# svohr/mixemt

Hardware: AMD Instinct MI355X
Metric: read x hap cells/sec through the EM iteration (EM iters/sec reported beside it as em_iters_per_s), 1000000 reads x 5408 haps in total, whole job (higher is better)
Workload: dtype f64

## Files before the change

### include/mixemt_hip_tuning.h

```cpp
#ifndef MIXEMT_HIP_TUNING_H
#define MIXEMT_HIP_TUNING_H

#include <stddef.h>
#include <stdint.h>

#ifdef __cplusplus
extern "C" {
#endif

struct mxm_em_state;

int mxm_reset_tuning(void);

int mxm_set_timing_events(void *ev_start, void *ev_stop);

int mxm_describe_stream_kernel(int32_t H, int32_t nb, char *buf, size_t len);

int mxm_diag_stream_read(const void *src, size_t bytes, int32_t wg_per_cu, int32_t blocked,
                         void *sink, void *stream);

struct mxm_coded;
int mxm_diag_stream_coded(const struct mxm_coded *c, int32_t H, int32_t wg_per_cu, void *sink, void *stream);

int mxm_diag_stream_quads(const struct mxm_coded *c, int32_t H, int32_t wg_per_cu, void *sink, void *stream);

int mxm_set_progress_callback(void (*fn)(const struct mxm_em_state *state_host, int32_t B, void *user),
                              void *user, int32_t every);

int mxm_set_loop_graph(int32_t mode);

int mxm_set_loop_fused(int32_t mode, int32_t chunk);

int mxm_set_fused_coded_grid(int32_t nwg);

int mxm_set_quad_left_grid(int32_t nwg);

int mxm_set_sparse_long_rows(int32_t on);
int mxm_set_sparse_long_entries(int32_t n);

int mxm_set_quad_encoder(int32_t kind);

int mxm_set_coded_batch_tile(int32_t bt);

int mxm_diag_fused_force_abort(int32_t on);

int mxm_diag_fused_stamps(const void *ws, unsigned long long *out_host);

int mxm_set_batch_tile(int32_t bt);

int mxm_set_compact_restarts(int32_t mode);

int mxm_set_min_rows_per_wg(int32_t n);

int mxm_set_sparse_max_distinct(int32_t n);

#ifdef __cplusplus
}
#endif
#endif
```

### mixemt_amd/_lib.py

```python

import ctypes
import os

_PKG = os.path.dirname(os.path.abspath(__file__))
LIB_PATH = os.environ.get("MXM_LIB") or os.path.join(_PKG, "lib", "libmixemt_hip.so")

c_i32, c_i64, c_f64 = ctypes.c_int32, ctypes.c_int64, ctypes.c_double
c_ptr, c_size = ctypes.c_void_p, ctypes.c_size_t


class EmState(ctypes.Structure):
    _fields_ = [("done", c_i32), ("iters", c_i32), ("l1", c_f64), ("ticket", ctypes.c_uint32), ("error", ctypes.c_uint32)]


class Coded(ctypes.Structure):
    _fields_ = [("rec", c_ptr), ("rec_off", c_ptr), ("ndist", c_ptr), ("R", c_i64),
                ("P_rest", c_ptr), ("ldp_rest", c_i64), ("w_rest", c_ptr), ("R_rest", c_i64),
                ("wide_rows", c_ptr), ("n_wide", c_i64),
                ("qrec", c_ptr), ("qoff", c_ptr), ("nquad", c_ptr), ("quad_rows", c_ptr), ("n_quad_rows", c_i64),
                ("byte_rows", c_ptr), ("n_byte_rows", c_i64)]


class AlnColumns(ctypes.Structure):
    _fields_ = [("n_aln", c_i64), ("n_frag", c_i64), ("ref_start", c_ptr), ("mapq", c_ptr), ("frag", c_ptr),
# ... 36 lines not shown
    "mxm_linearize": (ctypes.c_int, [c_ptr, c_i64, c_i64, c_i32, c_ptr, c_i64, c_ptr, c_ptr]),
    "mxm_em_iter": (ctypes.c_int, [c_ptr, c_i64, c_ptr, c_i64, c_ptr, c_ptr, c_ptr, c_i64, c_i32, c_i32,
                                   c_ptr, c_ptr, c_ptr, c_size, c_ptr]),
    "mxm_m_finalize": (ctypes.c_int, [c_ptr, c_ptr, c_ptr, c_ptr, c_i32, c_i32, c_f64, c_i32, c_ptr,
                                      c_ptr]),
    "mxm_em_loop": (ctypes.c_int, [c_ptr, c_i64, c_ptr, c_i64, c_ptr, c_i64, c_i32, c_i32,
                                   c_ptr, c_ptr, c_ptr, c_ptr, c_ptr, c_f64, c_i32, c_i32, c_ptr, c_size,
                                   c_ptr, ctypes.POINTER(EmState)]),
    "mxm_linearize_f32": (ctypes.c_int, [c_ptr, c_i64, c_i64, c_i32, c_ptr, c_i64, c_ptr, c_ptr]),
    "mxm_em_iter_f32": (ctypes.c_int, [c_ptr, c_i64, c_ptr, c_ptr, c_i64, c_i32, c_i32, c_ptr, c_ptr, c_ptr,
                                       c_size, c_ptr]),
    "mxm_em_loop_f32": (ctypes.c_int, [c_ptr, c_i64, c_ptr, c_i64, c_i32, c_i32, c_ptr, c_ptr, c_ptr, c_ptr,
                                       c_ptr, c_f64, c_i32, c_i32, c_ptr, c_size, c_ptr,
                                       ctypes.POINTER(EmState)]),
    "mxm_coded_bytes": (c_size, [c_i64, c_i32]),
    "mxm_exchange_handle_bytes": (c_size, []),
    "mxm_exchange_create": (ctypes.c_int, [c_i32, c_i32, c_i64, ctypes.POINTER(c_ptr), c_ptr]),
    "mxm_exchange_connect": (ctypes.c_int, [c_ptr, c_ptr]),
    "mxm_exchange_push": (ctypes.c_int, [c_ptr, c_ptr, c_i64, c_ptr]),
    "mxm_exchange_pull": (ctypes.c_int, [c_ptr, c_ptr, c_i64, c_ptr, c_i32, c_ptr]),
    "mxm_exchange_reduce": (ctypes.c_int, [c_ptr, c_ptr, c_i64, c_ptr, c_i32, c_ptr]),
    "mxm_exchange_info": (ctypes.c_int, [c_ptr, ctypes.POINTER(c_i32), ctypes.POINTER(c_i64)]),
    "mxm_exchange_destroy": (None, [c_ptr]),
    "mxm_expand_tables": (ctypes.c_int, [c_ptr, c_ptr, c_ptr, c_ptr, c_ptr, c_i32, c_i32, c_i64, c_ptr, c_ptr]),
    "mxm_quad_bytes": (c_size, [c_i64, c_i32]),
    "mxm_quad_lists_scratch_bytes": (c_size, [c_i64]),
    "mxm_quad_lists": (ctypes.c_int, [c_ptr, c_ptr, c_i64, c_ptr, c_ptr, c_ptr, c_ptr, c_size, c_ptr]),
    "mxm_build_quads": (ctypes.c_int, [ctypes.POINTER(Coded), c_i32, c_ptr, c_size, c_ptr, c_ptr, c_ptr, c_ptr]),
    "mxm_encode_rows": (ctypes.c_int, [c_ptr, c_i64, c_i64, c_i32, c_ptr, c_size, c_ptr, c_ptr, c_ptr, c_ptr, c_ptr]),
    "mxm_decode_rows": (ctypes.c_int, [ctypes.POINTER(Coded), c_i32, c_ptr, c_i64, c_ptr]),
    "mxm_row_argmax_votes_coded": (ctypes.c_int, [ctypes.POINTER(Coded), c_i32, c_i32, c_ptr, c_ptr, c_ptr, c_ptr, c_i64,
                                                  c_ptr, c_i64, c_ptr, c_ptr, c_ptr, c_ptr, c_size, c_ptr]),
    "mxm_em_step_coded": (ctypes.c_int, [ctypes.POINTER(Coded), c_i32, c_ptr, c_ptr, c_ptr, c_ptr, c_i64, c_ptr, c_i64,
                                         c_ptr, c_i64, c_i32, c_ptr]),
    "mxm_gather_columns_coded": (ctypes.c_int, [ctypes.POINTER(Coded), c_i32, c_ptr, c_i32, c_ptr, c_i64, c_ptr, c_i64,
                                                c_ptr, c_i64, c_ptr]),
    "mxm_em_iter_coded": (ctypes.c_int, [ctypes.POINTER(Coded), c_ptr, c_ptr, c_i32, c_i32, c_ptr, c_ptr, c_ptr,
                                         c_size, c_ptr]),
    "mxm_em_loop_coded": (ctypes.c_int, [ctypes.POINTER(Coded), c_ptr, c_i32, c_i32, c_ptr, c_ptr, c_ptr, c_ptr,
                                         c_ptr, c_f64, c_i32, c_i32, c_ptr, c_size, c_ptr,
                                         ctypes.POINTER(EmState)]),
    "mxm_em_step": (ctypes.c_int, [c_ptr, c_i64, c_ptr, c_ptr, c_i64, c_i32, c_ptr, c_i64, c_i32,
                                   c_ptr, c_ptr, c_size, c_ptr]),
    "mxm_log_normalize": (ctypes.c_int, [c_ptr, c_i32, c_ptr, c_ptr]),
    "mxm_l1_exp_diff": (ctypes.c_int, [c_ptr, c_ptr, c_i32, c_ptr, c_ptr]),
    "mxm_add_scalar": (ctypes.c_int, [c_ptr, c_i64, c_i64, c_i32, c_f64, c_ptr]),
    "mxm_assign_reads": (ctypes.c_int, [c_ptr, c_i64, c_ptr, c_ptr, c_i32, c_i64, c_i32, c_f64, c_ptr, c_ptr]),
    "mxm_diag_stream_read": (ctypes.c_int, [c_ptr, c_size, c_i32, c_i32, c_ptr, c_ptr]),
    "mxm_diag_stream_coded": (ctypes.c_int, [ctypes.POINTER(Coded), c_i32, c_i32, c_ptr, c_ptr]),
    "mxm_diag_stream_quads": (ctypes.c_int, [ctypes.POINTER(Coded), c_i32, c_i32, c_ptr, c_ptr]),
    "mxm_diag_fused_force_abort": (ctypes.c_int, [c_i32]),
    "mxm_set_fused_coded_grid": (ctypes.c_int, [c_i32]),
    "mxm_set_quad_left_grid": (ctypes.c_int, [c_i32]),
    "mxm_set_coded_batch_tile": (ctypes.c_int, [c_i32]),
    "mxm_set_sparse_long_rows": (ctypes.c_int, [c_i32]),
    "mxm_set_quad_encoder": (ctypes.c_int, [c_i32]),
    "mxm_set_sparse_long_entries": (ctypes.c_int, [c_i32]),
    "mxm_diag_fused_stamps": (ctypes.c_int, [c_ptr, ctypes.POINTER(ctypes.c_ulonglong)]),
    "mxm_set_timing_events": (ctypes.c_int, [c_ptr, c_ptr]),
    "mxm_set_batch_tile": (ctypes.c_int, [c_i32]),
    "mxm_encode_signatures": (ctypes.c_int64, [ctypes.c_char_p, c_ptr, c_i64, c_ptr, c_i64, c_ptr, c_ptr, c_ptr,
                                               c_i64]),
    "mxm_aln_encode": (ctypes.c_int, [ctypes.POINTER(AlnColumns), c_ptr, c_i64, c_ptr, c_i32, c_i32, c_i32, c_i32,
                                      ctypes.POINTER(c_ptr)]),
    "mxm_aln_sizes_of": (ctypes.c_int, [c_ptr, ctypes.POINTER(AlnSizes)]),
    "mxm_aln_fetch": (ctypes.c_int, [c_ptr, c_ptr, c_ptr, c_ptr, c_ptr, c_ptr, c_ptr, c_ptr, c_ptr, c_ptr]),
    "mxm_aln_fetch_fragments": (ctypes.c_int, [c_ptr, c_ptr, c_ptr, c_ptr, c_ptr]),
    "mxm_aln_free": (None, [c_ptr]),
    "mxm_bam_read": (ctypes.c_int, [ctypes.c_char_p, c_i32, ctypes.POINTER(c_ptr)]),
    "mxm_bam_sizes_of": (ctypes.c_int, [c_ptr, ctypes.POINTER(BamSizes)]),
    "mxm_bam_columns": (ctypes.c_int, [c_ptr, ctypes.POINTER(AlnColumns)]),
    "mxm_bam_fetch_names": (ctypes.c_int, [c_ptr, c_ptr, c_ptr, c_ptr, c_ptr]),
    "mxm_bam_free": (None, [c_ptr]),
    "mxm_observe_bases": (ctypes.c_int, [ctypes.POINTER(AlnColumns), c_ptr, c_i32, c_i32, c_i64, c_ptr, c_ptr]),
    "mxm_observe_bases_labelled": (ctypes.c_int, [ctypes.POINTER(AlnColumns), c_ptr, c_ptr, c_i32, c_i32, c_i32, c_i64,
                                                  c_ptr, c_ptr]),
    "mxm_consensus": (ctypes.c_int, [c_ptr, c_i32, c_i64, c_i64, c_i64, c_i32, c_ptr, c_ptr, c_ptr, c_ptr]),
    "mxm_new_variants": (ctypes.c_int, [c_ptr, c_i64, c_i32, ctypes.POINTER(c_i32), c_i32, c_i64, c_ptr, c_ptr, c_ptr]),
    "mxm_first_observed": (ctypes.c_int, [ctypes.POINTER(AlnColumns), c_ptr, c_ptr, c_i32, c_i32, c_i32, c_i64, c_ptr,
                                          c_ptr, c_ptr]),
    "mxm_extend_assign": (ctypes.c_int, [ctypes.POINTER(AlnColumns), c_ptr, c_ptr, c_i32, c_i32, ctypes.POINTER(c_i32),
                                         c_i32, c_i32, c_i32, c_i32, c_ptr, c_i64, c_ptr, c_ptr, c_ptr, c_ptr]),
    "mxm_set_compact_restarts": (ctypes.c_int, [c_i32]),
    "mxm_set_loop_graph": (ctypes.c_int, [c_i32]),
    "mxm_set_loop_fused": (ctypes.c_int, [c_i32, c_i32]),
    "mxm_set_progress_callback": (ctypes.c_int, [c_ptr, c_ptr, c_i32]),
    "mxm_set_min_rows_per_wg": (ctypes.c_int, [c_i32]),
    "mxm_reset_tuning": (ctypes.c_int, []),
    "mxm_describe_stream_kernel": (ctypes.c_int, [c_i32, c_i32, ctypes.c_char_p, c_size]),
    "mxm_set_sparse_max_distinct": (ctypes.c_int, [c_i32]),
    "mxm_row_argmax_votes": (ctypes.c_int, [c_ptr, c_i64, c_ptr, c_i64, c_i32, c_ptr, c_ptr,
                                            c_ptr, c_size, c_ptr]),
    "mxm_first_seen": (ctypes.c_int, [c_ptr, c_i64, c_i32, c_ptr, c_ptr]),
    "mxm_gather_columns": (ctypes.c_int, [c_ptr, c_i64, c_i64, c_i32, c_ptr, c_i32, c_ptr, c_i64, c_ptr]),
    "mxm_fold_logaddexp": (ctypes.c_int, [c_ptr, c_i64, ctypes.POINTER(c_ptr), ctypes.POINTER(c_i64), c_i32,
                                          c_i64, c_i32, c_f64, c_ptr]),
}

ABI_VERSION = 603

PROGRESS_FN = ctypes.CFUNCTYPE(None, ctypes.POINTER(EmState), c_i32, c_ptr)

_lib = None


class MixemtHipError(RuntimeError):
# ... 44 lines not shown
```

### mixemt_amd/csrc/common.hpp

```cpp
#ifndef MIXEMT_COMMON_HPP
#define MIXEMT_COMMON_HPP

typedef double d2 __attribute__((ext_vector_type(2)));

#define MXM_MAX_WG 1024
#define MXM_MAX_BT 4

struct mxm_slots {
    int s[MXM_MAX_BT];
};
#define MXM_LINEAR_MIN_H 65

static thread_local char g_err[512] = "";

static int fail(int code, const char *fmt, const char *a = "", long long b = 0, long long c = 0) {
    snprintf(g_err, sizeof(g_err), fmt, a, b, c);
    return code;
}
#define HIP_TRY(expr)                                                                        \
    do {                                                                                     \
        hipError_t e_ = (expr);                                                              \
        if (e_ != hipSuccess) return fail(-2, "HIP error: %s (line %lld)", hipGetErrorString(e_), __LINE__); \
    } while (0)

// ... 38 lines not shown
    return r;
}

template <int CTRL>
__device__ __forceinline__ double dpp_mov_f64(double v) {
    int lo = __double2loint(v), hi = __double2hiint(v);
    lo = __builtin_amdgcn_mov_dpp(lo, CTRL, 0xf, 0xf, true);
    hi = __builtin_amdgcn_mov_dpp(hi, CTRL, 0xf, 0xf, true);
    return __hiloint2double(hi, lo);
}
__device__ __forceinline__ double readlane_f64(double v, int src_lane) {
    const int lo = __builtin_amdgcn_readlane(__double2loint(v), src_lane);
    const int hi = __builtin_amdgcn_readlane(__double2hiint(v), src_lane);
    return __hiloint2double(hi, lo);
}
template <int CTRL, int ROW_MASK>
__device__ __forceinline__ double dpp_mov_old_f64(double old, double v) {
    int lo = __double2loint(v), hi = __double2hiint(v);
    lo = __builtin_amdgcn_update_dpp(__double2loint(old), lo, CTRL, ROW_MASK, 0xf, false);
    hi = __builtin_amdgcn_update_dpp(__double2hiint(old), hi, CTRL, ROW_MASK, 0xf, false);
    return __hiloint2double(hi, lo);
}
__device__ __forceinline__ double wave_sum_lane63(double v) {
    v += dpp_mov_f64<0xB1>(v);
    v += dpp_mov_f64<0x4E>(v);
    v += dpp_mov_f64<0x141>(v);
    v += dpp_mov_f64<0x140>(v);
    v += dpp_mov_old_f64<0x142, 0xA>(0.0, v);
    v += dpp_mov_old_f64<0x143, 0xC>(0.0, v);
    return v;
}
__device__ __forceinline__ double swap32_add(double x, double y) {
    typedef unsigned int u2s __attribute__((ext_vector_type(2)));
    const u2s lo = __builtin_amdgcn_permlane32_swap((unsigned)__double2loint(x), (unsigned)__double2loint(y), false, false);
    const u2s hi = __builtin_amdgcn_permlane32_swap((unsigned)__double2hiint(x), (unsigned)__double2hiint(y), false, false);
    return __hiloint2double((int)hi.x, (int)lo.x) + __hiloint2double((int)hi.y, (int)lo.y);
}
__device__ __forceinline__ double swap16_add(double x, double y) {
    typedef unsigned int u2s __attribute__((ext_vector_type(2)));
    const u2s lo = __builtin_amdgcn_permlane16_swap((unsigned)__double2loint(x), (unsigned)__double2loint(y), false, false);
    const u2s hi = __builtin_amdgcn_permlane16_swap((unsigned)__double2hiint(x), (unsigned)__double2hiint(y), false, false);
    return __hiloint2double((int)hi.x, (int)lo.x) + __hiloint2double((int)hi.y, (int)lo.y);
}
__device__ __forceinline__ double wave_sum3_by_row(double a, double b, double c) {
    const double ab = swap32_add(a, b);
    const double cc = swap32_add(c, c);
    double v = swap16_add(ab, cc);
    v += dpp_mov_f64<0xB1>(v);
    v += dpp_mov_f64<0x4E>(v);
    v += dpp_mov_f64<0x141>(v);
    v += dpp_mov_f64<0x140>(v);
    return v;
}
__device__ __forceinline__ double wave_max_lane63(double v) {
    v = fmax(v, dpp_mov_f64<0xB1>(v));
    v = fmax(v, dpp_mov_f64<0x4E>(v));
    v = fmax(v, dpp_mov_f64<0x141>(v));
    v = fmax(v, dpp_mov_f64<0x140>(v));
    v = fmax(v, dpp_mov_old_f64<0x142, 0xA>(v, v));
    v = fmax(v, dpp_mov_old_f64<0x143, 0xC>(v, v));
    return v;
}

__device__ __forceinline__ int wave_min_lane63_i32(int v) {
    v = min(v, __builtin_amdgcn_mov_dpp(v, 0xB1, 0xf, 0xf, true));
    v = min(v, __builtin_amdgcn_mov_dpp(v, 0x4E, 0xf, 0xf, true));
    v = min(v, __builtin_amdgcn_mov_dpp(v, 0x141, 0xf, 0xf, true));
    v = min(v, __builtin_amdgcn_mov_dpp(v, 0x140, 0xf, 0xf, true));
    v = min(v, __builtin_amdgcn_update_dpp(v, v, 0x142, 0xA, 0xf, false));
    v = min(v, __builtin_amdgcn_update_dpp(v, v, 0x143, 0xC, 0xf, false));
    return v;
}

__device__ __forceinline__ int wave_inclusive_scan_i32(int v) {
    v += __builtin_amdgcn_update_dpp(0, v, 0x111, 0xf, 0xf, false);
    v += __builtin_amdgcn_update_dpp(0, v, 0x112, 0xf, 0xf, false);
    v += __builtin_amdgcn_update_dpp(0, v, 0x114, 0xf, 0xf, false);
    v += __builtin_amdgcn_update_dpp(0, v, 0x118, 0xf, 0xf, false);
    v += __builtin_amdgcn_update_dpp(0, v, 0x142, 0xa, 0xf, false);
    v += __builtin_amdgcn_update_dpp(0, v, 0x143, 0xc, 0xf, false);
    return v;
}

__device__ __forceinline__ double weight_over_norm(double wr, double z) {
    if (z > 0.0) return wr / z;
    return (wr != 0.0) ? __builtin_nan("") : 0.0;
}

template <int NW, int N>
__device__ __forceinline__ void group_ratio_to_sgpr(const double *red, int lane, double num, double (&c)[N]) {
    static_assert(NW == 4 || NW == 8 || NW == 16, "waves per workgroup");
    static_assert(N * NW <= 64, "one partial per lane");
    double v = red[lane < N * NW ? lane : 0];
    v += dpp_mov_f64<0xB1>(v);
    v += dpp_mov_f64<0x4E>(v);
    if constexpr (NW >= 8) v += dpp_mov_f64<0x141>(v);
    if constexpr (NW == 16) v += dpp_mov_f64<0x140>(v);
    v = weight_over_norm(num, v);
#pragma unroll
    for (int g = 0; g < N; ++g) c[g] = readlane_f64(v, g * NW);
}

__device__ __forceinline__ double logaddexp_f64(double a, double b) {
    if (a == b) return a + 0.693147180559945309417232121458176568;
    double d = a - b;
    if (d > 0) return a + log1p(exp(-d));
// ... 26 lines not shown
```

### mixemt_amd/csrc/mixemt_hip.hip

```cpp
#include <hip/hip_runtime.h>
#include <stdint.h>
#include <stdio.h>
#include <stdlib.h>
#include <string.h>
#include <math.h>
#include <algorithm>
#include <atomic>
#include <mutex>
#include <type_traits>
#include <utility>
#include <vector>

#include "mixemt_hip.h"
#include "mixemt_hip_tuning.h"

#include "common.hpp"
#include "aln_encode.hpp"
#include "bam_reader.hpp"
#include "coded_kernels.hpp"
#include "quad_kernels.hpp"
#include "quad_batched_kernels.hpp"
#include "build_kernels.hpp"
#include "build_lut_kernels.hpp"
#include "build_sparse_kernels.hpp"
#include "em_kernels.hpp"
#include "estep_kernels.hpp"
#include "aux_kernels.hpp"
#include "records_kernels.hpp"
#include "fused_kernels.hpp"
#include "fused_cols_kernels.hpp"
#include "fused_coded_kernels.hpp"
#include "fused_narrow_kernels.hpp"
#include "exchange.hpp"
#include "observe_kernels.hpp"
#include "assemble_kernels.hpp"


struct mxm_em_state;
typedef void (*mxm_progress_fn)(const mxm_em_state *state_host, int32_t B, void *user);
struct mxm_tuning {
    int sparse_maxd = -1;
    int min_rows_per_wg = 8;
    int compact_restarts = 2;
    int max_bt = 4;
    int loop_graph = -1;
    int loop_fused = -1;
    int fused_chunk = 0;
    int fused_cols = 1;
    int fused_coded_wg = 0;
    int quad_left_wg = 0;
    int sparse_long_entries = 5120;
    int quad_encoder = 1;
    int sparse_long = 1;
    int coded_bt = 3;
    int fused_force_abort = 0;
    double fused_cells = 1.0e8;
    hipEvent_t ev_start = nullptr, ev_stop = nullptr;
    mxm_progress_fn progress = nullptr;
    void *progress_user = nullptr;
    int progress_every = 10;
};
static std::mutex g_tune_mu;
static mxm_tuning g_tune;
static thread_local mxm_tuning T;
#define MXM_ENTER() do { std::lock_guard<std::mutex> lk_(g_tune_mu); T = g_tune; } while (0)
template <typename F>
static int tune_set(F f) {
    std::lock_guard<std::mutex> lk(g_tune_mu);
    f(g_tune);
    return 0;
}
extern "C" int mxm_reset_tuning(void) {
    return tune_set([](mxm_tuning &t) { t = mxm_tuning(); });
}

static inline int clamp_grid(int64_t want, int cap) {
    if (want < 1) want = 1;
    return (int)(want < cap ? want : cap);
}

static inline int64_t part_ld(int H) { return ((int64_t)H + 1) & ~(int64_t)1; }

static hipError_t raise_dynamic_lds(const void *kernel, size_t bytes, const char *name) {
    const hipError_t e = hipFuncSetAttribute(kernel, hipFuncAttributeMaxDynamicSharedMemorySize, (int)bytes);
    if (e != hipSuccess)
        snprintf(g_err, sizeof(g_err), "%s: cannot opt into %zu bytes of dynamic LDS: %s", name, bytes,
                 hipGetErrorString(e));
    return e;
}

extern "C" int mxm_version(void) { return MXM_VERSION; }
extern "C" const char *mxm_last_error(void) { return g_err; }

extern "C" int mxm_linear_supported(int32_t H) {
    return (H >= MXM_LINEAR_MIN_H && H <= 8192) ? 1 : 0;
}

static size_t fused_sync_bytes() { return (sizeof(fused_sync) + 255) & ~(size_t)255; }
static size_t fused_snapshot_bytes(int H, int B) {
    return ((size_t)3 * B * H * sizeof(double) + (size_t)B * sizeof(mxm_em_state) + 255) & ~(size_t)255;
}
static size_t fused_rows_bytes(int H, int nwg) { return (size_t)(nwg + 2) * part_ld(H) * sizeof(double); }
// ... 288 lines not shown

extern "C" int mxm_linearize(const double *M, int64_t ldm, int64_t R, int32_t H, double *P, int64_t ldp,
                             double *rowmax, void *stream) {
    if (R < 0 || H <= 0) return fail(-1, "mxm_linearize: bad shape%s", "");
    if (ldm < H || ldp < H || (ldp & 1)) return fail(-1, "mxm_linearize: ldp must be even and >= H%s (ldp=%lld)", "", ldp);
    if (R == 0) return 0;
    if (wide_rows_ok(M, ldm, H) && (reinterpret_cast<uintptr_t>(P) & 15) == 0 &&
        linearize_wide<double>(M, ldm, R, (int)H, P, ldp, rowmax, (hipStream_t)stream) == 0) {
        HIP_TRY(hipGetLastError());
        return 0;
    }
    const int grid = clamp_grid(R, num_cu() * 8);
    hipLaunchKernelGGL(linearize_kernel, dim3(grid), dim3(ROW_THREADS), 0, (hipStream_t)stream, M, ldm, R,
                       (int)H, P, ldp, rowmax);
    HIP_TRY(hipGetLastError());
    return 0;
}

extern "C" int mxm_set_timing_events(void *ev_start, void *ev_stop) {
    return tune_set([=](mxm_tuning &t) { t.ev_start = (hipEvent_t)ev_start; t.ev_stop = (hipEvent_t)ev_stop; });
}

extern "C" int mxm_set_min_rows_per_wg(int32_t n) {
    if (n < 1) return fail(-1, "mxm_set_min_rows_per_wg: n < 1%s", "");
    return tune_set([n](mxm_tuning &t) { t.min_rows_per_wg = n; });
}

extern "C" int mxm_set_compact_restarts(int32_t mode) {
    return tune_set([mode](mxm_tuning &t) { t.compact_restarts = mode < 0 ? 0 : (mode > 2 ? 2 : mode); });
}

extern "C" int mxm_set_batch_tile(int32_t bt) {
    if (bt < 1 || bt > 4) return fail(-1, "mxm_set_batch_tile: tile must be 1..4%s", "");
    return tune_set([bt](mxm_tuning &t) { t.max_bt = bt; });
}

extern "C" int mxm_set_fused_coded_grid(int32_t nwg) {
    return tune_set([nwg](mxm_tuning &t) { t.fused_coded_wg = nwg > 0 ? nwg : 0; });
}

extern "C" int mxm_set_sparse_long_rows(int32_t on) {
    return tune_set([on](mxm_tuning &t) { t.sparse_long = on ? 1 : 0; });
}
extern "C" int mxm_set_sparse_long_entries(int32_t n) {
    return tune_set([n](mxm_tuning &t) { t.sparse_long_entries = n > 0 ? n : 0; });
}
extern "C" int mxm_set_coded_batch_tile(int32_t bt) {
    if (bt != 1 && bt != 3) return fail(-1, "mxm_set_coded_batch_tile: 1 or 3, got %s%lld", "", bt);
    return tune_set([bt](mxm_tuning &t) { t.coded_bt = bt; });
}
extern "C" int mxm_set_quad_encoder(int32_t kind) {
    if (kind != 0 && kind != 1) return fail(-1, "mxm_set_quad_encoder: 0 or 1, got %s%lld", "", kind);
    return tune_set([kind](mxm_tuning &t) { t.quad_encoder = kind; });
}
extern "C" int mxm_set_quad_left_grid(int32_t nwg) {
    return tune_set([nwg](mxm_tuning &t) { t.quad_left_wg = nwg > 0 ? nwg : 0; });
}

extern "C" int mxm_diag_fused_force_abort(int32_t on) {
    return tune_set([on](mxm_tuning &t) { t.fused_force_abort = on ? 1 : 0; });
}

#ifndef MXM_V1_THREADS
#define MXM_V1_THREADS 256
#endif
#ifndef MXM_V1_NBUF
#define MXM_V1_NBUF 2
#endif
#ifndef MXM_V1_WG_PER_CU
#define MXM_V1_WG_PER_CU 2
#endif
#ifndef MXM_V2_THREADS
#define MXM_V2_THREADS 512
#endif
#ifndef MXM_V2_NBUF
#define MXM_V2_NBUF 2
#endif
#ifndef MXM_V3_THREADS
#define MXM_V3_THREADS 512
#endif
#ifndef MXM_V3_NBUF
#define MXM_V3_NBUF 2
#endif
#ifndef MXM_V4_THREADS
#define MXM_V4_THREADS 512
#endif
#ifndef MXM_V4_NBUF
#define MXM_V4_NBUF 2
#endif
#ifndef MXM_V2_PREG
#define MXM_V2_PREG 1
#endif
#ifndef MXM_V3_PREG
#define MXM_V3_PREG 2
#endif
#ifndef MXM_V4_PREG
#define MXM_V4_PREG 2
#endif
#ifndef MXM_V1B_THREADS
#define MXM_V1B_THREADS 512
#endif
#ifndef MXM_V1B_NBUF
#define MXM_V1B_NBUF 3
#endif
#define MXM_MAX_COL2 4096
#define MXM_LDS_BUDGET (156 * 1024)
// ... 498 lines not shown
    return 0;
}

extern "C" int mxm_gather_columns_coded(const mxm_coded *c, int32_t H, const int32_t *cols, int32_t nC, const double *M_rest,
                                        int64_t ldm_rest, const int64_t *rest_rows, int64_t n_rest, double *out,
                                        int64_t ldo, void *stream) {
    int rc = coded_check(c, H, "mxm_gather_columns_coded");
    if (rc != 0) return rc;
    if (cols == nullptr || out == nullptr || nC <= 0 || ldo < nC) return fail(-1, "mxm_gather_columns_coded: bad arguments%s", "");
    if ((rc = rest_check("mxm_gather_columns_coded", H, M_rest, ldm_rest, rest_rows, n_rest)) != 0) return rc;
    const int64_t blocks = (c->R * nC + 255) / 256;
    hipLaunchKernelGGL(coded_gather_columns_kernel, dim3(clamp_grid(blocks, num_cu() * 16)), dim3(256), 0, (hipStream_t)stream,
                       c->rec, c->rec_off, c->ndist, coded_ld(H), c->R, cols, (int)nC, out, ldo);
    HIP_TRY(hipGetLastError());
    if (n_rest > 0) {
        hipLaunchKernelGGL(gather_columns_kernel, dim3(clamp_grid((n_rest * nC + 255) / 256, num_cu() * 16)), dim3(256), 0,
                           (hipStream_t)stream, M_rest, ldm_rest, n_rest, cols, (int)nC, out, ldo, rest_rows);
        HIP_TRY(hipGetLastError());
    }
    return 0;
}

struct coded_shape { int threads, nbuf, wg_per_cu; };
static const coded_shape g_coded_shapes[] = {{256, 4, 2}};
static const int g_coded_shape = 0;
template <int THREADS, int NBUF, int MINWG>
static int launch_coded(int nch, int nwg, hipStream_t stream, const mxm_coded *c, int ldc, const double *w, const double *props,
                        int H, double *partial, int64_t ldpart, const mxm_em_state *state, int run,
                        const int64_t *row_list = nullptr, int64_t n_list = 0, int part_row0 = 0) {
    switch (nch) {
#define COD_CASE(n) case n: if constexpr (n * THREADS <= 2048) { hipLaunchKernelGGL((em_iter_coded_kernel<THREADS, n, NBUF, MINWG>), dim3(nwg), dim3(THREADS), 0, stream, c->rec, c->rec_off, c->ndist, ldc, w, c->wide_rows, c->n_wide, props, c->R, H, partial, ldpart, state, run, row_list, n_list, c->nquad, part_row0); return 0; } break;
        COD_CASE(1) COD_CASE(2) COD_CASE(3) COD_CASE(4) COD_CASE(5) COD_CASE(6) COD_CASE(7) COD_CASE(8)
#undef COD_CASE
        default: break;
    }
    return fail(-1, "mxm_em_iter_coded: H=%s%lld outside the kernel's range", "", H);
}
#define QUAD_MAX_NCH 6
static int quad_left_share(const mxm_coded *c, int slots) {
    if (c->n_byte_rows <= 0 && c->n_wide <= 0) return 0;
    const double left_cost = 1.0 * (double)c->n_byte_rows + 1.5 * (double)c->n_wide;
    const double quad_cost = 0.67 * (double)c->n_quad_rows;
    int n = (int)((double)slots * left_cost / (left_cost + quad_cost) + 0.5);
    if (T.quad_left_wg > 0) n = T.quad_left_wg;
    if (n < 4) n = 4;
    if (n > slots / 2) n = slots / 2;
    const int64_t left = c->n_byte_rows > c->n_wide ? c->n_byte_rows : c->n_wide;
    n = clamp_grid(left, n);
    return n < 1 ? 1 : n;
}
static int launch_quad(int nch, int nwg, hipStream_t stream, const mxm_coded *c, const double *w, const double *props, int H,
                       double *partial, int64_t ldpart, const mxm_em_state *state, int run) {
    switch (nch) {
#define QUAD_CASE(n) case n: hipLaunchKernelGGL((em_iter_quad_kernel<n, 4>), dim3(nwg), dim3(QUAD_THREADS), 0, stream, c->qrec, c->qoff, c->nquad, c->quad_rows, c->n_quad_rows, c->R, w, props, H, partial, ldpart, 0, state, run); return 0;
        QUAD_CASE(1) QUAD_CASE(2) QUAD_CASE(3) QUAD_CASE(4) QUAD_CASE(5) QUAD_CASE(6)
#undef QUAD_CASE
        default: break;
    }
    return fail(-1, "mxm_em_iter_coded: H=%s%lld outside the quad kernel's range", "", H);
}
static int launch_quad_coded(int nch, int nwg, int nwg_left, hipStream_t stream, const mxm_coded *c, int ldc, const double *w,
                             const double *props, int H, double *partial, int64_t ldpart, const mxm_em_state *state, int run) {
    switch (nch) {
#define QC_CASE(n) case n: hipLaunchKernelGGL((em_iter_quad_coded_kernel<n, 4>), dim3(nwg), dim3(QUAD_THREADS), 0, stream, c->rec, c->rec_off, c->ndist, ldc, c->wide_rows, c->n_wide, c->byte_rows != nullptr ? c->byte_rows : c->quad_rows , c->n_byte_rows, c->qrec, c->qoff, c->nquad, c->quad_rows, c->n_quad_rows, c->R, w, props, H, partial, ldpart, nwg_left, state, run); return 0;
        QC_CASE(1) QC_CASE(2) QC_CASE(3) QC_CASE(4) QC_CASE(5) QC_CASE(6)
#undef QC_CASE
        default: break;
    }
    return fail(-1, "mxm_em_iter_coded: H=%s%lld outside the quad kernel's range", "", H);
}

static int em_iter_coded_one(const mxm_coded *c, const double *w, const double *props, int H, int run,
                             const mxm_em_state *state, double *colsum, double *partial, hipStream_t stream, bool timed,
                             const fin_args *fin = nullptr) {
    const int64_t ldpart = part_ld(H);
    const int ldc = coded_ld(H);
    const coded_shape sh = g_coded_shapes[g_coded_shape];
    const int nch = (ldc / 4 + sh.threads - 1) / sh.threads;
    int cap = num_cu() * sh.wg_per_cu;
    if (cap > MXM_MAX_WG - num_cu()) cap = MXM_MAX_WG - num_cu();
    if (cap < 1) cap = 1;
    const bool quads = c->qrec != nullptr && c->n_quad_rows > 0 && nch <= QUAD_MAX_NCH;
    int nwg_q = 0, nwg = 0;
    if (quads) {
        const int slots = cap < 2 * num_cu() ? cap : 2 * num_cu();
        const int nwg_b = quad_left_share(c, slots);
        nwg_q = clamp_grid((c->n_quad_rows + sh.nbuf - 1) / sh.nbuf, slots - nwg_b < 1 ? 1 : slots - nwg_b);
        nwg = nwg_q + nwg_b;
    } else {
        nwg = clamp_grid((c->R + sh.nbuf - 1) / sh.nbuf, cap);
    }
    if (timed && T.ev_start != nullptr) HIP_TRY(hipEventRecord(T.ev_start, stream));
    int *chk = reinterpret_cast<int *>(partial + (int64_t)MXM_MAX_WG * ldpart);
    int lrc;
    if (quads) {
        if (nwg > nwg_q) lrc = launch_quad_coded(nch, nwg, nwg - nwg_q, stream, c, ldc, w, props, H, partial, ldpart, state, run);
        else lrc = launch_quad(nch, nwg_q, stream, c, w, props, H, partial, ldpart, state, run);
        if (lrc != 0) return lrc;
    } else {
        lrc = launch_coded<256, 4, 2>(nch, nwg, stream, c, ldc, w, props, H, partial, ldpart, state, run);
        if (lrc != 0) return lrc;
    }
    HIP_TRY(hipGetLastError());
    if (timed && T.ev_stop != nullptr) HIP_TRY(hipEventRecord(T.ev_stop, stream));
    int nwg_rest = 0;
    mxm_slots sl;
    for (int i = 0; i < MXM_MAX_BT; ++i) sl.s[i] = run;
    if (c->R_rest > 0) {
        const int rc = stream_linear_tile(c->P_rest, c->ldp_rest, c->w_rest, props, c->R_rest, H, 1, sl, state,
                                          partial + (int64_t)nwg * ldpart, stream, false, &nwg_rest, MXM_MAX_WG - nwg,
                                          0 );
        if (rc != 0) return rc;
    }
    return reduce_tile(partial, nwg + nwg_rest, 1, H, colsum, state, sl, fin, stream, wide_check{chk, nwg, quads ? 0ll : (long long)c->n_wide});
}

#define QB_BT 3
// ... 1086 lines not shown
```

### mixemt_amd/csrc/quad_kernels.hpp

```cpp
#ifndef MIXEMT_QUAD_KERNELS_HPP
#define MIXEMT_QUAD_KERNELS_HPP

#define QUAD_MAX 256
#define QUAD_CODE_BYTES 2048
#define QUAD_HASH 1024
#define QUAD_THREADS 256
#define QUAD_CHUNK 65536ull

typedef unsigned int quad_u2 __attribute__((ext_vector_type(2)));
typedef unsigned int quad_u4 __attribute__((ext_vector_type(4)));
typedef double quad_d2 __attribute__((ext_vector_type(2)));

__global__ __launch_bounds__(QUAD_THREADS) void quad_encode_kernel(const uint8_t *__restrict__ rec,
                                                                   const int64_t *__restrict__ rec_off,
                                                                   const int32_t *__restrict__ ndist, int ldc, int H, int64_t R,
                                                                   uint8_t *__restrict__ qrec, unsigned long long qcap,
                                                                   int64_t *__restrict__ qoff, int32_t *__restrict__ nquad,
                                                                   unsigned long long *__restrict__ stats) {
#ifndef QUAD_RANK_BY_COUNT
#define QUAD_RANK_BY_COUNT 0
#endif
    __shared__ unsigned long long s_tab[QUAD_HASH];
    __shared__ int s_cnt[QUAD_RANK_BY_COUNT ? QUAD_HASH : 1];
    __shared__ int s_kcnt[QUAD_RANK_BY_COUNT ? QUAD_MAX : 1];
// ... 712 lines not shown
                    acc[k][e] = fma(cf, v[k][e], acc[k][e]);
                    asm volatile("" : "+v"(acc[k][e]));
                }
                lookup_quad(tbn, K, cw[jn]);
            }
        };
        upd(std::integral_constant<int, 0>{});
        upd(std::integral_constant<int, 1>{});
        upd(std::integral_constant<int, 2>{});
        upd(std::integral_constant<int, 3>{});
        upd(std::integral_constant<int, 4>{});
        upd(std::integral_constant<int, 5>{});
        upd(std::integral_constant<int, 6>{});
        upd(std::integral_constant<int, 7>{});
    };

    if (deal.nq > 0) {
        __syncthreads();
        fetch_meta(0, 0);
        __syncthreads();
        read_meta(0, 0);
        load_row(std::integral_constant<int, 0>{});
        read_meta(1, 0);
        load_row(std::integral_constant<int, 1>{});
        if constexpr (NBUF > 3) {
            read_meta(2, 0);
            load_row(std::integral_constant<int, 2>{});
        }
        if constexpr (NBUF > 4) {
            read_meta(3, 0);
            load_row(std::integral_constant<int, 3>{});
        }
        if constexpr (NBUF > 5) {
            read_meta(4, 0);
            load_row(std::integral_constant<int, 4>{});
        }
        publish(std::integral_constant<int, 0>{});
        __syncthreads();
        read_meta(NBUF - 1, 0);
        lookup_row(reinterpret_cast<const char *>(&s_tbl[0][0]), cw[0]);
        for (int64_t q = 0; q < deal.nq; q += NBUF) {
            step(std::integral_constant<int, 0>{}, q);
            step(std::integral_constant<int, 1>{}, q + 1);
            step(std::integral_constant<int, 2>{}, q + 2);
            if constexpr (NBUF > 3) step(std::integral_constant<int, 3>{}, q + 3);
            if constexpr (NBUF > 4) step(std::integral_constant<int, 4>{}, q + 4);
            if constexpr (NBUF > 5) step(std::integral_constant<int, 5>{}, q + 5);
        }
    }
    __syncthreads();
    *fault = s_fault;
}

template <int NCH, int NBUF>
__global__ __launch_bounds__(QUAD_THREADS, 2) void em_iter_quad_kernel(
    const uint8_t *__restrict__ qrec, const int64_t *__restrict__ qoff, const int32_t *__restrict__ nquad,
    const int64_t *__restrict__ quad_rows, int64_t n_rows, int64_t R, const double *__restrict__ w,
    const double *__restrict__ props, int H, double *__restrict__ partial, int64_t ldpart, int part_row0,
    const mxm_em_state *__restrict__ state, int run) {
    if (state != nullptr && state[run].done != 0) return;
    const int t = threadIdx.x;
    props += (int64_t)run * H;
    double p[NCH][4], acc[NCH][4];
#pragma unroll
    for (int k = 0; k < NCH; ++k) {
#pragma unroll
        for (int e = 0; e < 4; ++e) {
            const int c = 4 * (t + k * QUAD_THREADS) + e;
            p[k][e] = (c < H) ? props[c] : 0.0;
            acc[k][e] = 0.0;
        }
    }
    int fault = 0;
    quad_row_pass<NCH, NBUF, true>(qrec, qoff, nquad, quad_rows, n_rows, R, w, p, acc, &fault);
    const int64_t row = (int64_t)part_row0 + blockIdx.x;
    if (t == 0) {
        int *out = reinterpret_cast<int *>(partial + (int64_t)MXM_MAX_WG * ldpart) + 2 * row;
        out[0] = 0;
        out[1] = fault;
    }
    double *dst = partial + row * ldpart;
#pragma unroll
    for (int k = 0; k < NCH; ++k) {
        const int c = 4 * (t + k * QUAD_THREADS);
#pragma unroll
        for (int e = 0; e < 4; ++e)
            if (c + e < H) dst[c + e] = acc[k][e];
    }
}

template <int NCH, int NBUF>
__global__ __launch_bounds__(QUAD_THREADS, 2) void em_iter_quad_coded_kernel(
    const uint8_t *__restrict__ rec, const int64_t *__restrict__ rec_off, const int32_t *__restrict__ ndist, int ldc,
    const int64_t *__restrict__ wide_rows, int64_t n_wide, const int64_t *__restrict__ byte_rows, int64_t n_byte_rows,
    const uint8_t *__restrict__ qrec, const int64_t *__restrict__ qoff, const int32_t *__restrict__ nquad,
    const int64_t *__restrict__ quad_rows, int64_t n_quad_rows, int64_t R, const double *__restrict__ w,
    const double *__restrict__ props, int H, double *__restrict__ partial, int64_t ldpart, int nwg_left,
    const mxm_em_state *__restrict__ state, int run) {
    if (state != nullptr && state[run].done != 0) return;
    const int t = threadIdx.x;
    props += (int64_t)run * H;
    double p[NCH][4], acc[NCH][4];
#pragma unroll
    for (int k = 0; k < NCH; ++k) {
#pragma unroll
        for (int e = 0; e < 4; ++e) {
            const int c = 4 * (t + k * QUAD_THREADS) + e;
            p[k][e] = (c < H) ? props[c] : 0.0;
            acc[k][e] = 0.0;
        }
    }
    const int nwg_quad = (int)gridDim.x - nwg_left;
    int chk[2] = {0, 0};
    int64_t prow;
    if ((int)blockIdx.x < nwg_left) {
        bool meta_ready = false;
        coded_row_pass<QUAD_THREADS, NCH, NBUF, true, false, true, true>(rec, rec_off, ndist, ldc, w, wide_rows, n_wide, R, p, acc,
                                                                         meta_ready, chk, byte_rows, n_byte_rows, nquad,
                                                                         (int)blockIdx.x, nwg_left);
        prow = (int64_t)nwg_quad + blockIdx.x;
    } else {
        quad_row_pass<NCH, NBUF, true>(qrec, qoff, nquad, quad_rows, n_quad_rows, R, w, p, acc, &chk[1],
                                       (int)blockIdx.x - nwg_left, nwg_quad);
        prow = (int64_t)blockIdx.x - nwg_left;
    }
    if (t == 0) {
        int *out = reinterpret_cast<int *>(partial + (int64_t)MXM_MAX_WG * ldpart) + 2 * prow;
        out[0] = chk[0];
        out[1] = chk[1];
    }
    double *dst = partial + prow * ldpart;
#pragma unroll
    for (int k = 0; k < NCH; ++k) {
        const int c = 4 * (t + k * QUAD_THREADS);
#pragma unroll
        for (int e = 0; e < 4; ++e)
            if (c + e < H) dst[c + e] = acc[k][e];
    }
}

__global__ __launch_bounds__(QUAD_THREADS, 2) void diag_stream_quads_kernel(const uint8_t *__restrict__ qrec,
                                                                           const int64_t *__restrict__ qoff,
                                                                           const int32_t *__restrict__ nquad,
                                                                           const int64_t *__restrict__ quad_rows, int64_t n_rows,
                                                                           int64_t R, unsigned int *__restrict__ sink) {
    constexpr int NBUF = 4, THREADS = QUAD_THREADS;
    static_assert(THREADS % NBUF == 0, "a block of steps is a whole number of rounds");
    __shared__ long long s_off[2][THREADS];
    __shared__ int s_nd[2][THREADS];
    const int t = threadIdx.x;
    const row_deal deal(n_rows);
    if (deal.nq <= 0) return;
    quad_u2 x[NBUF];
    quad_u4 ya[NBUF], yb[NBUF];
    unsigned int acc = 0;
    auto fetch_meta = [&](int half, int64_t q0) {
        const int64_t q = q0 + t;
        const int64_t r = quad_rows[deal.row(q)];
        const bool ok = deal.live(q) && r >= 0 && r < R;
        const int nd = ok ? nquad[r] : 0;
        s_off[half][t] = nd > 0 && nd <= QUAD_MAX ? qoff[r] : 0;
        s_nd[half][t] = nd > 0 && nd <= QUAD_MAX ? nd : 0;
    };
    auto load_rec = [&](int slot, int64_t q) {
        const int half = (int)((q / THREADS) & 1), idx = (int)(q % THREADS);
        const long long off = s_off[half][idx];
        const int nd = __builtin_amdgcn_readfirstlane(s_nd[half][idx]);
        const int off_hi = __builtin_amdgcn_readfirstlane((int)(off >> 32)), off_lo = __builtin_amdgcn_readfirstlane((int)off);
        const uint8_t *base = qrec + (((long long)off_hi << 32) | (unsigned int)off_lo);
        const auto rs = __builtin_amdgcn_make_buffer_rsrc(const_cast<uint8_t *>(base), 0, nd > 0 ? QUAD_CODE_BYTES : 0, 0x00020000);
        x[slot] = __builtin_amdgcn_raw_buffer_load_b64(rs, t * 8, 0, 2);
        const auto rt = __builtin_amdgcn_make_buffer_rsrc(const_cast<uint8_t *>(base + QUAD_CODE_BYTES), 0, nd * 32, 0x00020000);
        ya[slot] = __builtin_amdgcn_raw_buffer_load_b128(rt, t * 32, 0, 2);
        yb[slot] = __builtin_amdgcn_raw_buffer_load_b128(rt, t * 32, 16, 2);
    };
    fetch_meta(0, 0);
    __syncthreads();
#pragma unroll
    for (int j = 0; j < NBUF - 1; ++j) load_rec(j, j);
    const int64_t nblk = (deal.nq + THREADS - 1) / THREADS;
    for (int64_t b = 0; b < nblk; ++b) {
        __syncthreads();
        fetch_meta((int)((b + 1) & 1), (b + 1) * THREADS);
        __syncthreads();
        for (int i = 0; i < THREADS; i += NBUF) {
#pragma unroll
            for (int j = 0; j < NBUF; ++j) {
// ... 10 lines not shown
```

Measured before the change: 871.5 billion.

## Process two quad-coded rows per step to halve barriers and reductions

Adds a quad_pair_pass that handles two reads per loop step in the quad-coded EM kernels, selected by a new default-on quad_row_group tuning knob. The two rows' dot products go through one combined wave reduction that splits the wave by halves, and they share a single __syncthreads and a double-buffered shared table. The aim is to amortise the per-row reduction and barrier latency that dominates the row-streaming loop. In exchange, register pressure roughly doubles for the v/table state, which may hurt occupancy under launch_bounds(…,2), and the existing kernels gain a GROUP template variant.

Result: no change. 871.3 billion (-0.0%).

```diff
diff --git a/include/mixemt_hip_tuning.h b/include/mixemt_hip_tuning.h
--- a/include/mixemt_hip_tuning.h
+++ b/include/mixemt_hip_tuning.h
@@ -35,6 +35,8 @@
 
 int mxm_set_quad_left_grid(int32_t nwg);
 
+int mxm_set_quad_row_group(int32_t rows);
+
 int mxm_set_sparse_long_rows(int32_t on);
 int mxm_set_sparse_long_entries(int32_t n);
 
diff --git a/mixemt_amd/_lib.py b/mixemt_amd/_lib.py
--- a/mixemt_amd/_lib.py
+++ b/mixemt_amd/_lib.py
@@ -112,6 +112,7 @@
     "mxm_diag_fused_force_abort": (ctypes.c_int, [c_i32]),
     "mxm_set_fused_coded_grid": (ctypes.c_int, [c_i32]),
     "mxm_set_quad_left_grid": (ctypes.c_int, [c_i32]),
+    "mxm_set_quad_row_group": (ctypes.c_int, [c_i32]),
     "mxm_set_coded_batch_tile": (ctypes.c_int, [c_i32]),
     "mxm_set_sparse_long_rows": (ctypes.c_int, [c_i32]),
     "mxm_set_quad_encoder": (ctypes.c_int, [c_i32]),
diff --git a/mixemt_amd/csrc/common.hpp b/mixemt_amd/csrc/common.hpp
--- a/mixemt_amd/csrc/common.hpp
+++ b/mixemt_amd/csrc/common.hpp
@@ -114,6 +114,15 @@
     v += dpp_mov_f64<0x140>(v);
     return v;
 }
+__device__ __forceinline__ double wave_sum2_by_half(double a, double b) {
+    double v = swap32_add(a, b);
+    v += dpp_mov_f64<0xB1>(v);
+    v += dpp_mov_f64<0x4E>(v);
+    v += dpp_mov_f64<0x141>(v);
+    v += dpp_mov_f64<0x140>(v);
+    v += dpp_mov_old_f64<0x142, 0xA>(0.0, v);
+    return v;
+}
 __device__ __forceinline__ double wave_max_lane63(double v) {
     v = fmax(v, dpp_mov_f64<0xB1>(v));
     v = fmax(v, dpp_mov_f64<0x4E>(v));
diff --git a/mixemt_amd/csrc/mixemt_hip.hip b/mixemt_amd/csrc/mixemt_hip.hip
--- a/mixemt_amd/csrc/mixemt_hip.hip
+++ b/mixemt_amd/csrc/mixemt_hip.hip
@@ -48,6 +48,7 @@
     int fused_chunk = 0;
     int fused_cols = 1;
     int fused_coded_wg = 0;
+    int quad_row_group = 2;
     int quad_left_wg = 0;
     int sparse_long_entries = 5120;
     int quad_encoder = 1;
@@ -442,6 +443,10 @@
 extern "C" int mxm_set_quad_encoder(int32_t kind) {
     if (kind != 0 && kind != 1) return fail(-1, "mxm_set_quad_encoder: 0 or 1, got %s%lld", "", kind);
     return tune_set([kind](mxm_tuning &t) { t.quad_encoder = kind; });
+}
+extern "C" int mxm_set_quad_row_group(int32_t rows) {
+    if (rows != 1 && rows != 2) return fail(-1, "mxm_set_quad_row_group: 1 or 2, got %s%lld", "", rows);
+    return tune_set([rows](mxm_tuning &t) { t.quad_row_group = rows; });
 }
 extern "C" int mxm_set_quad_left_grid(int32_t nwg) {
     return tune_set([nwg](mxm_tuning &t) { t.quad_left_wg = nwg > 0 ? nwg : 0; });
@@ -1046,7 +1051,7 @@
 static int launch_quad(int nch, int nwg, hipStream_t stream, const mxm_coded *c, const double *w, const double *props, int H,
                        double *partial, int64_t ldpart, const mxm_em_state *state, int run) {
     switch (nch) {
-#define QUAD_CASE(n) case n: hipLaunchKernelGGL((em_iter_quad_kernel<n, 4>), dim3(nwg), dim3(QUAD_THREADS), 0, stream, c->qrec, c->qoff, c->nquad, c->quad_rows, c->n_quad_rows, c->R, w, props, H, partial, ldpart, 0, state, run); return 0;
+#define QUAD_CASE(n) case n: if (T.quad_row_group == 2) hipLaunchKernelGGL((em_iter_quad_kernel<n, 4, 2>), dim3(nwg), dim3(QUAD_THREADS), 0, stream, c->qrec, c->qoff, c->nquad, c->quad_rows, c->n_quad_rows, c->R, w, props, H, partial, ldpart, 0, state, run); else hipLaunchKernelGGL((em_iter_quad_kernel<n, 4, 1>), dim3(nwg), dim3(QUAD_THREADS), 0, stream, c->qrec, c->qoff, c->nquad, c->quad_rows, c->n_quad_rows, c->R, w, props, H, partial, ldpart, 0, state, run); return 0;
         QUAD_CASE(1) QUAD_CASE(2) QUAD_CASE(3) QUAD_CASE(4) QUAD_CASE(5) QUAD_CASE(6)
 #undef QUAD_CASE
         default: break;
@@ -1056,7 +1061,7 @@
 static int launch_quad_coded(int nch, int nwg, int nwg_left, hipStream_t stream, const mxm_coded *c, int ldc, const double *w,
                              const double *props, int H, double *partial, int64_t ldpart, const mxm_em_state *state, int run) {
     switch (nch) {
-#define QC_CASE(n) case n: hipLaunchKernelGGL((em_iter_quad_coded_kernel<n, 4>), dim3(nwg), dim3(QUAD_THREADS), 0, stream, c->rec, c->rec_off, c->ndist, ldc, c->wide_rows, c->n_wide, c->byte_rows != nullptr ? c->byte_rows : c->quad_rows , c->n_byte_rows, c->qrec, c->qoff, c->nquad, c->quad_rows, c->n_quad_rows, c->R, w, props, H, partial, ldpart, nwg_left, state, run); return 0;
+#define QC_CASE(n) case n: if (T.quad_row_group == 2) hipLaunchKernelGGL((em_iter_quad_coded_kernel<n, 4, 2>), dim3(nwg), dim3(QUAD_THREADS), 0, stream, c->rec, c->rec_off, c->ndist, ldc, c->wide_rows, c->n_wide, c->byte_rows != nullptr ? c->byte_rows : c->quad_rows , c->n_byte_rows, c->qrec, c->qoff, c->nquad, c->quad_rows, c->n_quad_rows, c->R, w, props, H, partial, ldpart, nwg_left, state, run); else hipLaunchKernelGGL((em_iter_quad_coded_kernel<n, 4, 1>), dim3(nwg), dim3(QUAD_THREADS), 0, stream, c->rec, c->rec_off, c->ndist, ldc, c->wide_rows, c->n_wide, c->byte_rows != nullptr ? c->byte_rows : c->quad_rows , c->n_byte_rows, c->qrec, c->qoff, c->nquad, c->quad_rows, c->n_quad_rows, c->R, w, props, H, partial, ldpart, nwg_left, state, run); return 0;
         QC_CASE(1) QC_CASE(2) QC_CASE(3) QC_CASE(4) QC_CASE(5) QC_CASE(6)
 #undef QC_CASE
         default: break;
diff --git a/mixemt_amd/csrc/quad_kernels.hpp b/mixemt_amd/csrc/quad_kernels.hpp
--- a/mixemt_amd/csrc/quad_kernels.hpp
+++ b/mixemt_amd/csrc/quad_kernels.hpp
@@ -788,7 +788,167 @@
     *fault = s_fault;
 }
 
-template <int NCH, int NBUF>
+template <int NCH, bool NT>
+__device__ __forceinline__ void quad_pair_pass(const uint8_t *__restrict__ qrec, const int64_t *__restrict__ qoff,
+                                               const int32_t *__restrict__ nquad, const int64_t *__restrict__ quad_rows,
+                                               int64_t n_rows, int64_t R, const double *__restrict__ w,
+                                               const double (&p)[NCH][4], double (&acc)[NCH][4], int *fault, int vbid = -1,
+                                               int vgrid = 0) {
+    static_assert(NCH >= 1 && NCH <= 8, "eight code bytes per thread");
+    constexpr int THREADS = QUAD_THREADS, NW = THREADS / 64, AUX = NT ? 2 : 0;
+    static_assert(NW == 4 && THREADS % 4 == 0, "four wave sums per row; a pair never straddles a block of steps");
+    __shared__ __attribute__((aligned(16))) double s_tbl[2][2][QUAD_MAX * 4];
+    __shared__ __attribute__((aligned(16))) double red[2][2 * NW];
+    __shared__ long long s_off[2][THREADS];
+    __shared__ double s_wr[2][THREADS];
+    __shared__ int s_nd[2][THREADS];
+    __shared__ int s_fault;
+    const int t = threadIdx.x, lane = t & 63, wv = t >> 6;
+    const row_deal deal(n_rows, vbid >= 0 ? (int64_t)vbid : (int64_t)blockIdx.x, vbid >= 0 ? (int64_t)vgrid : (int64_t)gridDim.x);
+    if (t == 0) s_fault = 0;
+
+    auto fetch_meta = [&](int half, int64_t q0) {
+        const int64_t q = q0 + t;
+        const int64_t e = deal.row(q);
+        int64_t r = quad_rows[e];
+        int nd = 0;
+        if (r < 0 || r >= R || (e > 0 && quad_rows[e - 1] >= r)) {
+            s_fault = 1;
+            r = -1;
+        } else {
+            nd = nquad[r];
+            if (nd <= 0 || nd > QUAD_MAX) {
+                s_fault = 1;
+                nd = 0;
+            }
+        }
+        s_off[half][t] = (nd > 0) ? qoff[r] : 0;
+        s_nd[half][t] = nd;
+        s_wr[half][t] = (deal.live(q) && nd > 0) ? (w != nullptr ? w[r] : 1.0) : 0.0;
+    };
+    quad_u2 cw[2], cw_nx[2];
+    double tring[2][4];
+    int pre_off_lo[2], pre_off_hi[2], pre_nd[2];
+    double pre_wr;
+    auto read_meta = [&](int64_t q_load, int64_t q_weight) {
+        const int half = (int)((q_load / THREADS) & 1), idx = (int)(q_load % THREADS) + (lane & 1);
+        const long long off = s_off[half][idx];
+        const int nd = s_nd[half][idx];
+#pragma unroll
+        for (int i = 0; i < 2; ++i) {
+            pre_nd[i] = __builtin_amdgcn_readlane(nd, i);
+            pre_off_hi[i] = __builtin_amdgcn_readlane((int)(off >> 32), i);
+            pre_off_lo[i] = __builtin_amdgcn_readlane((int)off, i);
+        }
+        pre_wr = s_wr[(q_weight / THREADS) & 1][(q_weight % THREADS) + (lane >= NW ? 1 : 0)];
+    };
+    auto load_pair = [&]() {
+#pragma unroll
+        for (int i = 0; i < 2; ++i) {
+            const int nd = pre_nd[i];
+            const uint8_t *base = qrec + (((long long)pre_off_hi[i] << 32) | (unsigned int)pre_off_lo[i]);
+            const auto rs = __builtin_amdgcn_make_buffer_rsrc(const_cast<uint8_t *>(base), 0, nd > 0 ? QUAD_CODE_BYTES : 0, 0x00020000);
+            cw_nx[i] = __builtin_amdgcn_raw_buffer_load_b64(rs, t * 8, 0, AUX);
+            const auto rt = __builtin_amdgcn_make_buffer_rsrc(const_cast<uint8_t *>(base + QUAD_CODE_BYTES), 0, nd * 32, 0x00020000);
+            const quad_u4 a = __builtin_amdgcn_raw_buffer_load_b128(rt, t * 32, 0, AUX);
+            const quad_u4 b = __builtin_amdgcn_raw_buffer_load_b128(rt, t * 32, 16, AUX);
+            tring[i][0] = __hiloint2double((int)a.y, (int)a.x);
+            tring[i][1] = __hiloint2double((int)a.w, (int)a.z);
+            tring[i][2] = __hiloint2double((int)b.y, (int)b.x);
+            tring[i][3] = __hiloint2double((int)b.w, (int)b.z);
+        }
+    };
+    auto publish = [&](auto SLOT) {
+        constexpr int slot = decltype(SLOT)::value;
+#pragma unroll
+        for (int i = 0; i < 2; ++i) {
+            *reinterpret_cast<quad_d2 *>(&s_tbl[slot][i][t * 2]) = quad_d2{tring[i][0], tring[i][1]};
+            *reinterpret_cast<quad_d2 *>(&s_tbl[slot][i][QUAD_MAX * 2 + t * 2]) = quad_d2{tring[i][2], tring[i][3]};
+            cw[i] = cw_nx[i];
+        }
+    };
+    double v[2][NCH][4];
+    auto lookup_quad = [&](double (&dst)[NCH][4], const char *tb, auto K, const quad_u2 &c) {
+        constexpr int k = decltype(K)::value;
+        unsigned int off;
+        if constexpr (k < 4) off = quad_byte_x16<k>(c.x);
+        else off = quad_byte_x16<k - 4>(c.y);
+        const quad_d2 a = *reinterpret_cast<const quad_d2 *>(tb + off), b = *reinterpret_cast<const quad_d2 *>(tb + off + QUAD_MAX * 16);
+        dst[k][0] = a.x;
+        dst[k][1] = a.y;
+        dst[k][2] = b.x;
+        dst[k][3] = b.y;
+    };
+
+    auto step = [&](auto J, int64_t q) {
+        constexpr int j = decltype(J)::value, jn = j ^ 1;
+        if ((q % THREADS) == 0) fetch_meta((int)((q / THREADS + 1) & 1), q + THREADS);
+        const double wr = pre_wr;
+        double sab[2];
+#pragma unroll
+        for (int i = 0; i < 2; ++i) {
+            double s4[4] = {0.0, 0.0, 0.0, 0.0};
+#pragma unroll
+            for (int k = 0; k < NCH; ++k)
+#pragma unroll
+                for (int e = 0; e < 4; ++e) s4[e] = fma(v[i][k][e], p[k][e], s4[e]);
+            sab[i] = (s4[0] + s4[1]) + (s4[2] + s4[3]);
+            asm volatile("" : "+v"(sab[i]));
+        }
+        const double sa = sab[0], sb = sab[1];
+        __builtin_amdgcn_s_setprio(1);
+        const double z2 = wave_sum2_by_half(sa, sb);
+        if ((lane & 31) == 31) red[j][(lane >> 5) * NW + wv] = z2;
+        publish(std::integral_constant<int, jn>{});
+        load_pair();
+        __syncthreads();
+        read_meta(q + 6, q + 2);
+        double z = red[j][lane < 2 * NW ? lane : 0];
+        z += dpp_mov_f64<0xB1>(z);
+        z += dpp_mov_f64<0x4E>(z);
+        const double cfv = weight_over_norm(wr, z);
+        const double cf[2] = {readlane_f64(cfv, 0), readlane_f64(cfv, NW)};
+        __builtin_amdgcn_s_setprio(0);
+        auto upd = [&](auto I, auto K) {
+            constexpr int i = decltype(I)::value, k = decltype(K)::value;
+            if constexpr (k < NCH) {
+#pragma unroll
+                for (int e = 0; e < 4; ++e) {
+                    acc[k][e] = fma(cf[i], v[i][k][e], acc[k][e]);
+                    asm volatile("" : "+v"(acc[k][e]));
+                }
+                lookup_quad(v[i], reinterpret_cast<const char *>(&s_tbl[jn][i][0]), K, cw[i]);
+            }
+        };
+        quad_static_for<8>([&](auto K) { upd(std::integral_constant<int, 0>{}, K); });
+        quad_static_for<8>([&](auto K) { upd(std::integral_constant<int, 1>{}, K); });
+    };
+
+    if (deal.nq > 0) {
+        __syncthreads();
+        fetch_meta(0, 0);
+        __syncthreads();
+        read_meta(0, 0);
+        load_pair();
+        publish(std::integral_constant<int, 0>{});
+        read_meta(2, 0);
+        load_pair();
+        __syncthreads();
+        read_meta(4, 0);
+        quad_static_for<NCH>([&](auto K) {
+            lookup_quad(v[0], reinterpret_cast<const char *>(&s_tbl[0][0][0]), K, cw[0]);
+            lookup_quad(v[1], reinterpret_cast<const char *>(&s_tbl[0][1][0]), K, cw[1]);
+        });
+        for (int64_t q = 0; q < deal.nq; q += 4) {
+            step(std::integral_constant<int, 0>{}, q);
+            step(std::integral_constant<int, 1>{}, q + 2);
+        }
+    }
+    __syncthreads();
+    *fault = s_fault;
+}
+
+template <int NCH, int NBUF, int GROUP>
 __global__ __launch_bounds__(QUAD_THREADS, 2) void em_iter_quad_kernel(
     const uint8_t *__restrict__ qrec, const int64_t *__restrict__ qoff, const int32_t *__restrict__ nquad,
     const int64_t *__restrict__ quad_rows, int64_t n_rows, int64_t R, const double *__restrict__ w,
@@ -808,8 +968,12 @@
         }
     }
     int fault = 0;
-    quad_row_pass<NCH, NBUF, true>(qrec, qoff, nquad, quad_rows, n_rows, R, w, p, acc, &fault);
+    static_assert(GROUP == 1 || GROUP == 2, "rows per step");
+    if constexpr (GROUP == 2) quad_pair_pass<NCH, true>(qrec, qoff, nquad, quad_rows, n_rows, R, w, p, acc, &fault);
+    else quad_row_pass<NCH, NBUF, true>(qrec, qoff, nquad, quad_rows, n_rows, R, w, p, acc, &fault);
     const int64_t row = (int64_t)part_row0 + blockIdx.x;
+    int tc = t;
+    asm volatile("" : "+v"(tc));
     if (t == 0) {
         int *out = reinterpret_cast<int *>(partial + (int64_t)MXM_MAX_WG * ldpart) + 2 * row;
         out[0] = 0;
@@ -818,14 +982,14 @@
     double *dst = partial + row * ldpart;
 #pragma unroll
     for (int k = 0; k < NCH; ++k) {
-        const int c = 4 * (t + k * QUAD_THREADS);
+        const int c = 4 * (tc + k * QUAD_THREADS);
 #pragma unroll
         for (int e = 0; e < 4; ++e)
             if (c + e < H) dst[c + e] = acc[k][e];
     }
 }
 
-template <int NCH, int NBUF>
+template <int NCH, int NBUF, int GROUP>
 __global__ __launch_bounds__(QUAD_THREADS, 2) void em_iter_quad_coded_kernel(
     const uint8_t *__restrict__ rec, const int64_t *__restrict__ rec_off, const int32_t *__restrict__ ndist, int ldc,
     const int64_t *__restrict__ wide_rows, int64_t n_wide, const int64_t *__restrict__ byte_rows, int64_t n_byte_rows,
@@ -856,10 +1020,17 @@
                                                                          (int)blockIdx.x, nwg_left);
         prow = (int64_t)nwg_quad + blockIdx.x;
     } else {
-        quad_row_pass<NCH, NBUF, true>(qrec, qoff, nquad, quad_rows, n_quad_rows, R, w, p, acc, &chk[1],
-                                       (int)blockIdx.x - nwg_left, nwg_quad);
+        static_assert(GROUP == 1 || GROUP == 2, "rows per step");
+        if constexpr (GROUP == 2)
+            quad_pair_pass<NCH, true>(qrec, qoff, nquad, quad_rows, n_quad_rows, R, w, p, acc, &chk[1], (int)blockIdx.x - nwg_left,
+                                      nwg_quad);
+        else
+            quad_row_pass<NCH, NBUF, true>(qrec, qoff, nquad, quad_rows, n_quad_rows, R, w, p, acc, &chk[1],
+                                           (int)blockIdx.x - nwg_left, nwg_quad);
         prow = (int64_t)blockIdx.x - nwg_left;
     }
+    int tc = t;
+    asm volatile("" : "+v"(tc));
     if (t == 0) {
         int *out = reinterpret_cast<int *>(partial + (int64_t)MXM_MAX_WG * ldpart) + 2 * prow;
         out[0] = chk[0];
@@ -868,7 +1039,7 @@
     double *dst = partial + prow * ldpart;
 #pragma unroll
     for (int k = 0; k < NCH; ++k) {
-        const int c = 4 * (t + k * QUAD_THREADS);
+        const int c = 4 * (tc + k * QUAD_THREADS);
 #pragma unroll
         for (int e = 0; e < 4; ++e)
             if (c + e < H) dst[c + e] = acc[k][e];
```
